# ubisoft/ubisoft-laforge-msmd

Hardware: AMD Instinct MI355X
Metric: FLAME frames/sec on 4s@16kHz clips (whole job; MSMD.forward motion-coefficient frames) (higher is better)
Workload: dtype bf16; 1 GPU; configs[1]: MSMD.forward, batch=32 x 4 s clips per GPU, wav2vec2-base encoder + 8-layer motion decoder, eval-mode, synthetic closed-form weights; batch_per_gpu=32, frames_per_clip=100, parallelism=dp1 (independent clips, no collective), launch=one hipGraph replay per step (the batch sits in the captured input buffers)

## Files before the change

include/msmd_hip.h:

```cpp
#ifndef MSMD_HIP_H
#define MSMD_HIP_H

#include <stdint.h>

#ifdef __cplusplus
extern "C" {
#endif

#define MSMD_F32 0
#define MSMD_BF16 1
#define MSMD_F16 2
#define MSMD_F16X2 3

#define MSMD_ACT_NONE 0
#define MSMD_ACT_GELU 1
#define MSMD_ACT_ELU 2

typedef void* msmd_stream_t;

int msmd_abi_version(void);
#define MSMD_GEMM_VARIANT(v) ((v) << 8)
#define MSMD_GEMM_WRITE_THROUGH (1 << 16)
#define MSMD_GEMM_PAIRED_STORES (1 << 17)
#define MSMD_GEMM_STAGGER (1 << 18)
// ... 105 lines not shown
                                    long q_bstride, long q_tstride, long k_bstride, long k_tstride, long v_bstride,
                                    long v_tstride, long o_bstride, long o_tstride, float scale, const uint8_t* mask,
                                    float p_drop, const unsigned long* rng_state, unsigned int site, int dtype,
                                    const void* const* prefetch_ptrs, const long* prefetch_bytes, int n_prefetch,
                                    msmd_stream_t stream);

int msmd_dropout(const void* x, const void* residual, void* y, long n, float p, const unsigned long* rng_state,
                 unsigned int site, int dtype, msmd_stream_t stream);

int msmd_attention_bwd(const void* Q, const void* K, const void* V, const void* dO, void* dQ, void* dK, void* dV,
                       int B, int H, int Tq, int Tk, long q_bstride, long q_tstride, long k_bstride,
                       long k_tstride, long v_bstride, long v_tstride, long do_bstride, long do_tstride,
                       long dq_bstride, long dq_tstride, long dk_bstride, long dk_tstride, long dv_bstride,
                       long dv_tstride, float scale, const uint8_t* mask, float p_drop,
                       const unsigned long* rng_state, unsigned int site, msmd_stream_t stream);

int msmd_pad_audio(const float* audio, float* out, int B, int L, int reflect_len, int replicate_len,
                   msmd_stream_t stream);

#define MSMD_CONV0_SPLITS 16
int msmd_conv0_stats(const float* audio, const float* w0, float* stats, double* ws, int B, int L, int reflect_len,
                     int replicate_len, int C, float eps, msmd_stream_t stream);

int msmd_conv0_gn_gelu(const float* audio, const float* w0, const float* stats, const float* gamma,
                       const float* beta, void* out, int B, int L, int reflect_len, int replicate_len,
                       int C, int out_dtype, msmd_stream_t stream);

int msmd_conv0_ln_gelu(const float* audio, const float* w0, const float* bias, const float* gamma, const float* beta,
                       void* out, int B, int L, int reflect_len, int replicate_len, int C, float eps, int out_dtype,
                       msmd_stream_t stream);

int msmd_interp_linear(const void* x, void* y, int B, int T_in, int T_crop, int T_out, int C, int dtype,
                       msmd_stream_t stream);

int msmd_group_pad(const void* x, void* y, int B, int T, int G, int Cg, int Cg_out, int pad, int dtype, int out_dtype,
                   msmd_stream_t stream);

int msmd_pos_conv(const void* x, const void* w, const float* bias, void* y, int B, int T, int G, int Cg, int kpos,
                  int dtype, msmd_stream_t stream);

int msmd_denoiser_pack_input(const float* motion, const float* eps, const float* c0, const float* c1,
                             const float* prev_motion, const float* indicator, void* feats, int N, int L,
                             int Lp, int dm, int Kpad, int motion_batch, int out_dtype, msmd_stream_t stream);

int msmd_denoiser_pack_input_guided(const float* motion, const float* eps, const float* c0, const float* c1,
                                    const float* prev_motion, const float* indicator, const unsigned char* guide_mask,
                                    const float* guide_values, void* feats, int N, int L, int Lp, int dm, int Kpad,
                                    int motion_batch, int out_dtype, msmd_stream_t stream);

int msmd_denoiser_prepare(const float* motion, const float* eps, const float* t0, const float* t1, const long* ts,
                          int n_steps, const float* prev_motion, long prev_motion_stride, const float* indicator,
                          void* feats, int N, int L, int Lp, int dm, int Kpad, const float* person_a, int cols_a,
                          const float* person_b, int cols_b, void* pf, int kp_person, const float* style,
                          long style_n, void* style_out, const void* emb_table, void* emb, int d,
                          const float* prev_audio, long prev_audio_stride, int Lpa, void* mem, long mem_stride,
                          int dtype, msmd_stream_t stream);
// ... 348 lines not shown
```

ubisoft-laforge-msmd_amd/csrc/audio.hip:

```cpp
#include "common.h"

__device__ __forceinline__ int pad_src(int j, int L, int r, int rep) {
  const int L1 = L + 2 * r, L2 = L1 + 2 * r;
  j -= rep;
  j = j < 0 ? 0 : (j >= L2 ? L2 - 1 : j);
  if (r > 0) {
    j -= r;
    j = j < 0 ? -j : (j >= L1 ? 2 * (L1 - 1) - j : j);
    j -= r;
    j = j < 0 ? -j : (j >= L ? 2 * (L - 1) - j : j);
  }
  return j;
}

__global__ void pad_audio_kernel(const float* __restrict__ a, float* __restrict__ out, int L, int Lp, int r, int rep) {
  const int b = blockIdx.y;
  for (int j = blockIdx.x * blockDim.x + threadIdx.x; j < Lp; j += gridDim.x * blockDim.x)
    out[(long)b * Lp + j] = a[(long)b * L + pad_src(j, L, r, rep)];
}

extern "C" int msmd_pad_audio(const float* audio, float* out, int B, int L, int reflect_len, int replicate_len,
                              msmd_stream_t stream) {
  if (B <= 0 || L <= 0 || reflect_len < 0 || replicate_len < 0 || reflect_len >= L) return 1;
  const int Lp = L + 4 * reflect_len + 2 * replicate_len;
  dim3 grid(min((Lp + 255) / 256, 1024), B), block(256);
  hipLaunchKernelGGL(pad_audio_kernel, grid, block, 0, (hipStream_t)stream, audio, out, L, Lp, reflect_len,
                     replicate_len);
  MSMD_RETURN_LAST();
}

#define C0_K 10
#define C0_S 5
#define C0_SPLITS 16
#define C0_NMOM 66

static bool conv0_geometry_ok(int B, int L, int reflect_len, int replicate_len) {
  if (B <= 0 || L <= 0 || reflect_len < 0 || replicate_len < 0 || reflect_len >= L) return false;
  return (long)L + 4L * reflect_len + 2L * replicate_len >= C0_K;
}


__global__ __launch_bounds__(256) void conv0_moments_partial(const float* __restrict__ audio, double* __restrict__ ws,
                                                             int L, int r, int rep, int T0, int pass) {
  __shared__ double red[4][C0_NMOM];
  const int b = blockIdx.y, split = blockIdx.x;
  const int per = (T0 + C0_SPLITS - 1) / C0_SPLITS;
  const int t_begin = split * per, t_end = min(T0, t_begin + per);
  double* out = ws + ((long)b * C0_SPLITS + split) * C0_NMOM;
  const float* xa = audio + (long)b * L;
  const int n_used = T0 * C0_S + C0_K - C0_S;
  const int n_mu = min(256, n_used);
  {
    const int j = (int)(((long)threadIdx.x * n_used) / n_mu);
    double v = threadIdx.x < n_mu ? (double)xa[pad_src(j, L, r, rep)] : 0.0;
    for (int o = 32; o > 0; o >>= 1) v += __shfl_xor(v, o, 64);
    if ((threadIdx.x & 63) == 0) red[threadIdx.x >> 6][0] = v;
    __syncthreads();
  }
  const float mu = (float)((red[0][0] + red[1][0] + red[2][0] + red[3][0]) / (double)n_mu);
  if (threadIdx.x == 0) out[0] = (double)mu;
  float m[C0_NMOM];
#pragma unroll
  for (int i = 0; i < C0_NMOM; ++i) m[i] = 0.f;
  for (int t = t_begin + threadIdx.x; t < t_end; t += 256) {
    float x[C0_K];
#pragma unroll
    for (int k = 0; k < C0_K; ++k) x[k] = xa[pad_src(t * C0_S + k, L, r, rep)] - mu;
#pragma unroll
    for (int k = 0; k < C0_K; ++k) {
      m[1 + k] += x[k];
#pragma unroll
      for (int k2 = k; k2 < C0_K; ++k2) {
        const int idx = 1 + C0_K + k * C0_K - (k * (k - 1)) / 2 + (k2 - k);
        m[idx] = fmaf(x[k], x[k2], m[idx]);
      }
    }
  }
#pragma unroll
  for (int i = 1; i < C0_NMOM; ++i) {
    double v = (double)m[i];
    for (int o = 32; o > 0; o >>= 1) v += __shfl_xor(v, o, 64);
    if ((threadIdx.x & 63) == 0) red[threadIdx.x >> 6][i] = v;
  }
  __syncthreads();
  if (threadIdx.x >= 1 && threadIdx.x < C0_NMOM)
    out[threadIdx.x] = red[0][threadIdx.x] + red[1][threadIdx.x] + red[2][threadIdx.x] + red[3][threadIdx.x];
}

__global__ void conv0_stats_finish(const double* __restrict__ ws, const float* __restrict__ w0,
                                   float* __restrict__ stats, int C, int T0, float eps) {
  __shared__ double mom[C0_NMOM];
  const int b = blockIdx.y;
  if (threadIdx.x < C0_NMOM) {
    double v = 0.0;
    for (int s = 0; s < C0_SPLITS; ++s) v += ws[((long)b * C0_SPLITS + s) * C0_NMOM + threadIdx.x];
    mom[threadIdx.x] = v;
  }
  __syncthreads();
  const int c = blockIdx.x * blockDim.x + threadIdx.x;
  if (c >= C) return;
  const double mu = ws[(long)b * C0_SPLITS * C0_NMOM];
  double w[C0_K], wsum = 0.0, ws1 = 0.0, q = 0.0;
  for (int k = 0; k < C0_K; ++k) { w[k] = (double)w0[c * C0_K + k]; wsum += w[k]; ws1 += w[k] * mom[1 + k]; }
  int idx = 1 + C0_K;
  for (int k = 0; k < C0_K; ++k)
    for (int k2 = k; k2 < C0_K; ++k2) q += (k2 == k ? 1.0 : 2.0) * w[k] * w[k2] * mom[idx++];
  const double mc = ws1 / T0;
  const double var = q / T0 - mc * mc;
  stats[((long)b * C + c) * 2 + 0] = (float)(mc + mu * wsum);
  stats[((long)b * C + c) * 2 + 1] = (float)(1.0 / sqrt(fmax(var, 0.0) + (double)eps));
}

extern "C" int msmd_conv0_stats(const float* audio, const float* w0, float* stats, double* ws, int B, int L,
                                int reflect_len, int replicate_len, int C, float eps, msmd_stream_t stream) {
  if (!conv0_geometry_ok(B, L, reflect_len, replicate_len) || C <= 0 || !ws) return 1;
  const int Lp = L + 4 * reflect_len + 2 * replicate_len;
  const int T0 = (Lp - C0_K) / C0_S + 1;
  hipStream_t st = (hipStream_t)stream;
  dim3 grid(C0_SPLITS, B);
  hipLaunchKernelGGL(conv0_moments_partial, grid, dim3(256), 0, st, audio, ws, L, reflect_len, replicate_len, T0, 1);
  hipLaunchKernelGGL(conv0_stats_finish, dim3((C + 255) / 256, B), dim3(256), 0, st, ws, w0, stats, C, T0, eps);
  MSMD_RETURN_LAST();
}

template <typename TO, bool SPLIT = false>
__global__ __launch_bounds__(256) void conv0_gn_gelu_kernel(const float* __restrict__ audio,
                                                            const float* __restrict__ w0,
                                                            const float* __restrict__ stats,
                                                            const float* __restrict__ gamma,
                                                            const float* __restrict__ beta, TO* __restrict__ out,
                                                            int L, int r, int rep, int C, int T0) {
  constexpr int FR = 64;
  __shared__ float xs[FR * C0_S + C0_K];
  const int b = blockIdx.y, t0 = blockIdx.x * FR;
  const int nt = min(FR, T0 - t0);
  const int ns = nt * C0_S + (C0_K - C0_S);
  for (int i = threadIdx.x; i < ns; i += 256) xs[i] = audio[(long)b * L + pad_src(t0 * C0_S + i, L, r, rep)];
  __syncthreads();
  const int grp = threadIdx.x >> 6, q = threadIdx.x & 63;
  for (int c0 = q * 8; c0 < C; c0 += 512) {
    float w[8][C0_K], sc[8], sh[8];
#pragma unroll
    for (int e = 0; e < 8; ++e) {
      const int c = c0 + e;
#pragma unroll
// ... 210 lines not shown
    }
  }
}

extern "C" int msmd_conv0_ln_gelu(const float* audio, const float* w0, const float* bias, const float* gamma,
                                  const float* beta, void* out, int B, int L, int reflect_len, int replicate_len,
                                  int C, float eps, int out_dtype, msmd_stream_t stream) {
  if (!conv0_geometry_ok(B, L, reflect_len, replicate_len) || C != 512) return 1;
  const int Lp = L + 4 * reflect_len + 2 * replicate_len;
  const int T0 = (Lp - C0_K) / C0_S + 1;
  dim3 grid((T0 + 63) / 64, B), block(256);
  return dispatch_dtype<float, f16_t, bf16_t>(out_dtype, [&](auto tag) {
    typedef MSMD_TAG_T(tag) TO;
    hipLaunchKernelGGL(conv0_ln_gelu_kernel<TO>, grid, block, 0, (hipStream_t)stream, audio, w0, bias, gamma, beta,
                       (TO*)out, L, reflect_len, replicate_len, T0, eps);
    MSMD_RETURN_LAST();
  });
}

template <typename T>
__global__ void interp_linear_kernel(const T* __restrict__ x, T* __restrict__ y, int T_in, int T_crop, int T_out,
                                     int C) {
  const int b = blockIdx.z, j = blockIdx.y;
  const float scale = (float)T_crop / (float)T_out;
  float src = fmaf(scale, (float)j + 0.5f, -0.5f);
  src = src < 0.f ? 0.f : src;
  int i0 = (int)src;
  i0 = i0 < T_crop - 1 ? i0 : T_crop - 1;
  const int i1 = i0 + 1 < T_crop ? i0 + 1 : T_crop - 1;
  const float w1 = src - (float)i0, w0 = 1.0f - w1;
  const T* p0 = x + ((long)b * T_in + i0) * C;
  const T* p1 = x + ((long)b * T_in + i1) * C;
  T* q = y + ((long)b * T_out + j) * C;
  for (int c = blockIdx.x * blockDim.x + threadIdx.x; c < C; c += gridDim.x * blockDim.x) {
#pragma clang fp contract(off)
    const float a0 = w0 * to_f32(p0[c]), a1 = w1 * to_f32(p1[c]);
    q[c] = from_f32<T>(a0 + a1);
  }
}

extern "C" int msmd_interp_linear(const void* x, void* y, int B, int T_in, int T_crop, int T_out, int C, int dtype,
                                  msmd_stream_t stream) {
  if (B <= 0 || T_in <= 0 || T_crop <= 0 || T_crop > T_in || T_out <= 0 || C <= 0) return 1;
  dim3 grid((C + 255) / 256, T_out, B), block(256);
  return dispatch_dtype<float, f16_t, bf16_t>(dtype, [&](auto tag) {
    typedef MSMD_TAG_T(tag) T;
    hipLaunchKernelGGL(interp_linear_kernel<T>, grid, block, 0, (hipStream_t)stream, (const T*)x, (T*)y, T_in, T_crop,
                       T_out, C);
    MSMD_RETURN_LAST();
  });
}

template <typename T, bool SPLIT>
__global__ void group_pad_kernel(const T* __restrict__ x, void* __restrict__ yv, int Tn, int G, int Cg, int Cgo,
                                 int pad) {
  const int b = blockIdx.z, g = blockIdx.y;
  const int Tp = Tn + 2 * pad;
  const long n = (long)Tp * Cgo;
  for (long i = blockIdx.x * blockDim.x + threadIdx.x; i < n; i += (long)gridDim.x * blockDim.x) {
    const int tp = (int)(i / Cgo), c = (int)(i % Cgo);
    const int t = tp - pad;
// ... 33 lines not shown
```

ubisoft-laforge-msmd_amd/csrc/common.h:

```cpp
#pragma once
#include <hip/hip_runtime.h>
#include <stdint.h>

#include "../../include/msmd_hip.h"

typedef __bf16 bf16_t;
typedef __bf16 bf16x8 __attribute__((ext_vector_type(8)));
typedef __bf16 bf16x4 __attribute__((ext_vector_type(4)));
typedef __bf16 bf16x2 __attribute__((ext_vector_type(2)));
typedef _Float16 f16_t;
typedef _Float16 f16x8 __attribute__((ext_vector_type(8)));
typedef _Float16 f16x4 __attribute__((ext_vector_type(4)));
typedef _Float16 f16x2 __attribute__((ext_vector_type(2)));
typedef float f32x4 __attribute__((ext_vector_type(4)));
typedef float f32x2 __attribute__((ext_vector_type(2)));
typedef float f32x16 __attribute__((ext_vector_type(16)));
typedef uint32_t u32x4 __attribute__((ext_vector_type(4)));
typedef uint32_t u32x2 __attribute__((ext_vector_type(2)));

struct __attribute__((packed, aligned(4))) F3 { float x, y, z; };
struct __attribute__((packed, aligned(4))) I3 { int a, b, c; };

#define MSMD_WAVE 64

// ... 162 lines not shown
}
__device__ __forceinline__ double wave_sum_f64(double v) {
#pragma unroll
  for (int o = 32; o > 0; o >>= 1) v += __shfl_xor(v, o, 64);
  return v;
}
__device__ __forceinline__ float wave_max(float v) {
#pragma unroll
  for (int o = 32; o > 0; o >>= 1) v = fmaxf(v, __shfl_xor(v, o, 64));
  return v;
}

__device__ __forceinline__ float block_sum(float v, float* red) {
  v = wave_sum(v);
  const int lane = threadIdx.x & 63, wid = threadIdx.x >> 6, nw = blockDim.x >> 6;
  __syncthreads();
  if (lane == 0) red[wid] = v;
  __syncthreads();
  float t = 0.f;
  for (int i = 0; i < nw; ++i) t += red[i];
  return t;
}

template <typename T> struct Elems16;
template <> struct Elems16<float> { static constexpr int n = 4; };
template <> struct Elems16<bf16_t> { static constexpr int n = 8; };
template <> struct Elems16<f16_t> { static constexpr int n = 8; };

template <typename T> struct TypeTag { typedef T type; };
template <typename T> struct DtypeCode;
template <> struct DtypeCode<float> { static constexpr int value = MSMD_F32; };
template <> struct DtypeCode<bf16_t> { static constexpr int value = MSMD_BF16; };
template <> struct DtypeCode<f16_t> { static constexpr int value = MSMD_F16; };
template <typename... Ts, typename F>
static int dispatch_dtype(int dtype, F&& f) {
  int r = 1;
  (void)((dtype == DtypeCode<Ts>::value && ((r = f(TypeTag<Ts>{})), true)) || ...);
  return r;
}
#define MSMD_TAG_T(tag) typename decltype(tag)::type
template <typename TI, typename TO> constexpr bool kStoragePair = sizeof(TI) == 4 || sizeof(TO) == 4 || __is_same(TI, TO);
```

ubisoft-laforge-msmd_amd/csrc/gemm.hip:

```cpp
#include "gemm_tiles.h"
#include <atomic>
#include <utility>

struct GemmArgs {
  const void* A; const void* W; const float* bias; const void* R; void* C;
  int M, N, K;
  long lda; int rows_per_batch; long a_batch_stride; long ldw, ldc, ldr;
  int act; int vec_ok; float inv_rpb;
  long strideA, strideW, strideC, strideBias, strideR;
  int mt, nt;
  int batch_inner; long strideA2, strideW2, strideC2;
  void* Z; float p_drop; const unsigned long* rng; unsigned site;
  int xn;
  int flags;
  const float* a_stats = nullptr; int a_nt = 0; const float* w_colsum = nullptr;
  const float* r_stats = nullptr; int r_nt = 0; const float* r_gamma = nullptr; const float* r_beta = nullptr;
  float* stats_out = nullptr; float ln_eps = 1e-5f;
  int stagger_ticks = 0;
};

enum : int {
  GF_WRITE_THROUGH = 1, GF_PAIRED_STORES = 2, GF_STAGGER = 4,
  GF_ACT_BWD = 8,
  GF_ONE_TILE = 16, GF_NO_256 = 32,
// ... 1990 lines not shown

extern "C" int msmd_gemm_actbwd(const void* A, const void* W, const void* Z, void* C, int M, int N, int K, int in_dtype, int out_dtype, long lda,
                                long ldw, int act, float p_drop, const unsigned long* rng_state, unsigned int site, msmd_stream_t stream) {
  if (!Z || in_dtype != out_dtype || (in_dtype != MSMD_BF16 && in_dtype != MSMD_F16) || (N & 3) || ((uintptr_t)Z & 7)) return 1;
  if (K % 64) return 1;
  GemmCall c;
  c.A = A; c.W = W; c.C = C; c.M = M; c.N = N; c.K = K; c.in_dtype = in_dtype; c.out_dtype = out_dtype;
  c.lda = lda; c.ldw = ldw; c.ldc = N; c.act = act & (0xffff | MSMD_GEMM_WRITE_THROUGH | MSMD_GEMM_PAIRED_STORES);
  c.z_out = const_cast<void*>(Z); c.p_drop = p_drop; c.rng = rng_state; c.site = site; c.internal_flags = GF_ACT_BWD;
  return gemm_run(gemm_plan, c, stream);
}

extern "C" int msmd_gemm_batched2(const void* A, const void* W, void* C, int M, int N, int K, int in_dtype, int out_dtype, long lda, long ldw,
                                  long ldc, int batch_outer, long strideA_o, long strideW_o, long strideC_o, int batch_inner, long strideA_i,
                                  long strideW_i, long strideC_i, msmd_stream_t stream) {
  GemmCall c;
  c.A = A; c.W = W; c.C = C; c.M = M; c.N = N; c.K = K; c.in_dtype = in_dtype; c.out_dtype = out_dtype;
  c.lda = lda; c.ldw = ldw; c.ldc = ldc; c.act = MSMD_ACT_NONE;
  c.batch = batch_outer; c.strideA = strideA_o; c.strideW = strideW_o; c.strideC = strideC_o;
  c.batch_inner = batch_inner; c.strideA2 = strideA_i; c.strideW2 = strideW_i; c.strideC2 = strideC_i;
  return gemm_run(gemm_plan, c, stream);
}

static bool conv_chain_table(ChainTable& t, int B, int T0, int C, int N, int n, const int* kernel, const int* stride, int flags) {
  if (B <= 0 || T0 <= 0 || C <= 0 || N <= 0 || n < 2 || n > 4 || !kernel || !stride || (N % 256)) return false;
  t = ChainTable{};
  t.n = n; t.nt = N / 256;
  t.per_block = (flags & MSMD_CONV_CHAIN_ROW_BLOCK_TICKETS) != 0;
  t.release = (flags & MSMD_CONV_CHAIN_RELEASE) != 0;
  long t_in = T0, c_in = C;
  int tickets = 0, counters = 0;
  for (int l = 0; l < n; ++l) {
    ChainProblem& q = t.pr[l];
    if (kernel[l] <= 0 || stride[l] <= 0 || t_in < kernel[l]) return false;
    const long t_out = (t_in - kernel[l]) / stride[l] + 1, M = (long)B * t_out, K = kernel[l] * c_in;
    if ((K % 64) || K < 128 || M >= (1L << 24)) return false;
    q.M = (int)M; q.K = (int)K; q.rows_per_batch = (int)t_out; q.inv_rpb = 1.0f / (float)t_out;
    q.lda = stride[l] * c_in; q.a_batch_stride = t_in * c_in;
    q.t_in = (int)t_in; q.stride = stride[l]; q.taps = kernel[l];
    q.mt = (int)((M + 255) / 256);
    q.ticket0 = tickets; q.cnt0 = counters;
    tickets += t.per_block ? q.mt : q.mt * t.nt;
    counters += q.mt;
    if (((long)(B - 1) * q.a_batch_stride + (t_out - 1) * q.lda + K) * 2 >= (1L << 32) || (long)N * K * 2 >= (1L << 32)) return false;
    t_in = t_out; c_in = N;
  }
// ... 58 lines not shown
```

ubisoft-laforge-msmd_amd/model.py:

```python
from __future__ import annotations

from types import SimpleNamespace

import torch
import torch.nn as nn

from . import init, ops, shapes, synth
from .blocks import Rows, add, materialise, norm, project
from .utils.model_common import ParamTree, PositionalEncoding, enc_dec_mask, sinusoid_table


def _cd(args) -> torch.dtype:
    name = getattr(args, "compute_dtype", "bf16")
    if name in ("bf16", torch.bfloat16):
        return torch.bfloat16
    if name in ("fp32", "float32", torch.float32):
        return torch.float32
    if name in ("f16x2", "split"):
        return torch.float32
    if name in ("fp16", "float16", "half", torch.float16):
        return torch.float16
    raise ValueError(f"Unknown compute dtype {name}!")


# ... 528 lines not shown
    @torch.no_grad()
    def extract_audio_768_feature(self, audio, frame_num=None):
        frame_num = frame_num or self.n_motions
        return self._audio_768(audio, frame_num, self.compute_dtype).float()

    @torch.no_grad()
    def forward(self, motion_feat, audio_or_feat, shape_feat, style_feat=None, prev_motion_feat=None,
                prev_audio_feat=None, time_step=None, indicator=None, train_with_CFG=True, keep_separate=False,
                eps=None):
        dtype = self.compute_dtype
        if self.use_style:
            assert style_feat is not None, "Missing style features!"
        batch_size = motion_feat.shape[0]
        net = self.denoising_net
        fused = net.prepares_fused(dtype) and not self.training
        if prev_audio_feat is None:
            prev_audio_feat = self.start_audio_feat.expand(batch_size, -1, -1)
        mem = None
        if audio_or_feat.ndim == 2:
            assert audio_or_feat.shape[1] == 16000 * self.n_motions / self.fps, \
                f"Incorrect audio length {audio_or_feat.shape[1]}"
            if fused:
                La, Lpa, d = self.n_motions, prev_audio_feat.shape[1], net.feature_dim
                h = self._audio_768(audio_or_feat, La, dtype)
                mem = torch.empty(batch_size, Lpa + La, d, device=self.device, dtype=dtype)
                audio_cd = mem[:, Lpa:]
                ops.gemm(h, *self._afm_packed(dtype), out=audio_cd, M=La, N=d, K=h.shape[-1], lda=h.shape[-1], ldc=d,
                         batch=batch_size, strideA=La * h.shape[-1], strideW=0, strideC=(Lpa + La) * d)
            else:
                audio_cd = self._audio_feat(audio_or_feat, self.n_motions, dtype)
            audio_feat_saved = audio_cd.float()
        elif audio_or_feat.ndim == 3:
            assert audio_or_feat.shape[1] == self.n_motions, f"Incorrect audio feature length {audio_or_feat.shape[1]}"
            audio_feat_saved = audio_or_feat
        else:
            raise ValueError(f"Incorrect audio input shape {audio_or_feat.shape}")
        audio_feat = audio_feat_saved
        if audio_or_feat.ndim != 2:
            audio_cd = None
        if shape_feat.ndim == 2:
            shape_feat = shape_feat.unsqueeze(1)
        if style_feat is not None and style_feat.ndim == 2:
            style_feat = style_feat.unsqueeze(1)
        if prev_motion_feat is None:
            prev_motion_feat = self.start_motion_feat.expand(batch_size, -1, -1)
        if len(self.guiding_conditions) > 0 and train_with_CFG:
            assert len(self.guiding_conditions) <= 2, "Only support 1 or 2 CFG conditions!"
            if len(self.guiding_conditions) == 1 or self.cfg_mode == "independent":
                null_cond_prob = 0.5 if len(self.guiding_conditions) >= 2 else 0.1
                if "style" in self.guiding_conditions:
                    mask_style = torch.rand(batch_size, device=self.device) < null_cond_prob
                    style_feat = torch.where(mask_style.view(-1, 1, 1),
                                             self.null_style_feat.expand(batch_size, -1, -1), style_feat)
                if "audio" in self.guiding_conditions:
# ... 130 lines not shown
```

ubisoft-laforge-msmd_amd/ops.py:

```python
from __future__ import annotations

import ctypes
import functools
import math
import os

import numpy as np
import torch
from torch.autograd.function import once_differentiable

from . import _lib

_HEADER = _lib.parse_constants()


def _h(*names):
    vals = tuple(_HEADER["MSMD_" + n] for n in names)
    return vals if len(vals) > 1 else vals[0]


F32, BF16, F16, F16X2 = _h("F32", "BF16", "F16", "F16X2")
SPLIT = "f16x2"


# ... 541 lines not shown

def dynamic_threshold_(res, L, ratio, dt_min, dt_max):
    _need_cuda(res)
    if res.dtype != torch.float32 or not res.is_contiguous():
        raise TypeError("dynamic_threshold_ takes a contiguous fp32 tensor")
    N, T_all, C = res.shape
    _lib.check(_lib.load().msmd_dynamic_threshold(_p(res), N, T_all, L, C, float(ratio), float(dt_min), float(dt_max),
                                                  _stream()), "msmd_dynamic_threshold")
    return res


def pad_audio(audio, reflect_len, replicate_len):
    lib = _lib.load()
    B, L = audio.shape
    out = torch.empty(B, L + 4 * reflect_len + 2 * replicate_len, device=audio.device, dtype=torch.float32)
    _lib.check(lib.msmd_pad_audio(_p(audio), _p(out), B, L, reflect_len, replicate_len, _stream()), "msmd_pad_audio")
    return out


def conv0_workspace(B, device):
    return torch.empty(B, CONV0_SPLITS, 66, device=device, dtype=torch.float64)


def conv0_gn_gelu(audio, w0, gamma, beta, reflect_len, replicate_len, out_dtype, eps=1e-5):
    lib = _lib.load()
    B, L = audio.shape
    C = w0.shape[0]
    Lp = L + 4 * reflect_len + 2 * replicate_len
    T0 = (Lp - 10) // 5 + 1
    stats = torch.empty(B, C, 2, device=audio.device, dtype=torch.float32)
    ws = conv0_workspace(B, audio.device)
    _lib.check(lib.msmd_conv0_stats(_p(audio), _p(w0), _p(stats), _p(ws), B, L, reflect_len, replicate_len, C, eps,
                                    _stream()), "msmd_conv0_stats")
    out = empty((B, T0, C), audio.device, out_dtype)
    _lib.check(lib.msmd_conv0_gn_gelu(_p(audio), _p(w0), _p(stats), _p(gamma), _p(beta), _p(out), B, L, reflect_len,
                                      replicate_len, C, _dt(out), _stream()), "msmd_conv0_gn_gelu")
    return out


def conv0_ln_gelu(audio, w0, bias, gamma, beta, reflect_len, replicate_len, out_dtype, eps=1e-5):
    lib = _lib.load()
    B, L = audio.shape
    C = w0.shape[0]
    Lp = L + 4 * reflect_len + 2 * replicate_len
    T0 = (Lp - 10) // 5 + 1
    out = torch.empty(B, T0, C, device=audio.device, dtype=out_dtype)
    _lib.check(lib.msmd_conv0_ln_gelu(_p(audio), _p(w0), _p(bias), _p(gamma), _p(beta), _p(out), B, L, reflect_len,
                                      replicate_len, C, eps, _dt(out), _stream()), "msmd_conv0_ln_gelu")
    return out


def interp_linear(x, t_out, t_crop=None):
    lib = _lib.load()
    B, T, C = x.shape
    t_crop = T if t_crop is None else min(int(t_crop), T)
    y = torch.empty(B, t_out, C, device=x.device, dtype=x.dtype)
    _lib.check(lib.msmd_interp_linear(_p(x), _p(y), B, T, t_crop, t_out, C, _dt(x), _stream()), "msmd_interp_linear")
    return y


def group_pad(x, groups, pad, cg_out=None, split=False):
    lib = _lib.load()
    B, T, C = x.shape
    cg = C // groups
    cg_out = cg if cg_out is None else cg_out
    y = empty((B, groups, T + 2 * pad, cg_out), x.device, SPLIT if split else x.dtype)
    _lib.check(lib.msmd_group_pad(_p(x), _p(y), B, T, groups, cg, cg_out, pad, _dt(x), _dt(y), _stream()),
               "msmd_group_pad")
    return y


def pos_conv(x, w, bias, groups, kpos=128):
    lib = _lib.load()
    _need_cuda(x)
    B, T, C = x.shape
    cg = C // groups
    if not (x.is_contiguous() and w.is_contiguous() and w.dtype == x.dtype and tuple(w.shape) == (groups, cg, kpos * cg)):
        raise TypeError("pos_conv takes contiguous x (B, T, G*Cg) and w (G, Cg, kpos*Cg) of one 16-bit dtype")
    if bias.dtype != torch.float32 or bias.numel() != C:
        raise TypeError("pos_conv takes an fp32 bias of G*Cg values")
    y = torch.empty_like(x)
# ... 1732 lines not shown
```

ubisoft-laforge-msmd_amd/training_script.py:

```python
from __future__ import annotations

import contextlib
import os

import numpy as np
import torch

from . import autograd as ag
from . import dp, ops, synth
from . import train_graph as tg


def load_loss_weights(args, device=None):
    w = {"noise": 1.0, "vert": float(args.l_vert), "vel": float(args.l_vel), "smooth": float(args.l_smooth),
         "head_angle": float(args.l_head_angle), "head_vel": float(args.l_head_vel),
         "head_smooth": float(args.l_head_smooth), "head_trans": float(args.l_head_trans)}
    if not args.use_vertex_space:
        w["vel"] *= 4.5e-8
        w["smooth"] *= 4e-7
    legacy = args.dataset_type[:9] == "HDTF_TFHP" or args.dataset_type == "flame_mead_ravdess"
    if not legacy and args.use_vertex_space:
        w["vert"] *= 1e-7
        w["vel"] *= 1e-7
        w["smooth"] *= 2e-8
# ... 290 lines not shown
            motion_in = ops.truncate_rows_(motion.float().clone().contiguous(), e32, 1, self.pad_replicate)
            indicator = (torch.arange(args.n_motions, device=self.device).expand(B, -1) < end_idx.unsqueeze(1)).float()
        else:
            audio_in, motion_in = audio, motion
            indicator = torch.ones(B, args.n_motions, device=self.device)
        ts = draws["t"][i] if "t" in draws else model.diffusion_sched.uniform_sample_t_device(B)
        eps = draws["eps"][i] if "eps" in draws else torch.randn_like(motion_in)
        ns, na = self._cfg_masks(draws, i, B)
        shape_in = torch.zeros_like(shape) if getattr(args, "do_ignore_shape", False) else shape
        return dict(style=style, end_idx=end_idx, audio_in=audio_in, motion_in=motion_in, indicator=indicator, ts=ts, eps=eps,
                    ns=ns, na=na, shape_in=shape_in)

    def _hand_off(self, batch, W0, audio_feat, dtype):
        model, n_prev = self.model, self.args.n_prev_motions
        if W0["end_idx"] is None:
            return W0["motion_in"][:, -n_prev:].detach(), audio_feat[:, -n_prev:].detach()
        audio = batch[0][0]
        with torch.no_grad():
            if ag.TrainNoise.active:
                prev_audio = tg.audio_feat_train(model, audio, model.n_motions, dtype).float()[:, -n_prev:]
            else:
                enc = model.audio_encoder
                chain, enc.conv_chain = enc.conv_chain, False
                try:
                    prev_audio = model.extract_audio_feature(audio)[:, -n_prev:]
                finally:
                    enc.conv_chain = chain
        return batch[1][0][:, -n_prev:], prev_audio

    def _loss_terms(self, i, W, target, prev_motion, shape, mu, logvar, terms, lw):
        args = self.args
        prev = prev_motion if i == 1 else None
        if self.vertex_space:
            pairs = tg.loss_vert_train(args, i == 0, shape, W["motion_in"], target, prev, self.coef_stats, self.flame,
                                       W["end_idx"]).items()
        else:
            tup = tg.loss_no_vert_train(args, i == 0, W["motion_in"], target, prev, W["end_idx"],
                                        halve=False)
            pairs = zip(("noise", "vel", "smooth", "head_angle", "head_vel", "head_smooth", "head_trans"),
                        [(v, 0.5) for v in tup[:6]] + [(tup[6], 1.0)])
        for key, val in pairs:
            val, sc = val if isinstance(val, tuple) else (val, 1.0)
            if val is not None and torch.is_tensor(val) and lw.get(key, 0) > 0:
                terms[key].append((val, sc))
        terms["kl_div"].append((tg.kl_train(mu, logvar), 1.0))

    def _two_windows_batched(self, batch, draws, trunc, cross, lw, dtype):
        model, se = self.model, self.style_enc
        audio_pair, motion_pair, shape = batch
        B = audio_pair[0].shape[0]
# ... 446 lines not shown
```

ubisoft-laforge-msmd_amd/utils/wav2vec2.py:

```python
from __future__ import annotations

from types import SimpleNamespace

import torch
import torch.nn as nn

from .. import ops, shapes, synth
from ..blocks import Rows, add, materialise, norm, project
from .model_common import ParamTree, pad_audio_plan

CONV_KERNEL = shapes.CONV_KERNEL
CONV_STRIDE = shapes.CONV_STRIDE


def compute_mask_indices(shape, mask_prob, mask_length, min_masks=0, rng=None):
    import numpy as np
    rng = np.random if rng is None else rng
    bsz, T = shape
    n_mask = max(min_masks, int(mask_prob * T / float(mask_length) + rng.rand()))
    spans = []
    for _ in range(bsz):
        lengths = np.full(n_mask, mask_length)
        if lengths.sum() == 0:
            lengths[0] = min(mask_length, T - 1)
# ... 85 lines not shown
            snap = os.path.join(repo, "snapshots", open(ref).read().strip())
            if _is_checkpoint_dir(snap):
                return snap
        for snap in sorted(glob.glob(os.path.join(repo, "snapshots", "*"))):
            if _is_checkpoint_dir(snap):
                return snap
    return None


def load_hf_state_dict(directory):
    import os
    st = os.path.join(directory, "model.safetensors")
    if os.path.isfile(st):
        from safetensors.torch import load_file
        return load_file(st, device="cpu")
    sd = torch.load(os.path.join(directory, "pytorch_model.bin"), map_location="cpu", weights_only=True)
    return sd.get("state_dict", sd) if isinstance(sd, dict) else sd


class Wav2Vec2Model(nn.Module):

    model_type = "wav2vec2"
    conv_chain = True

    def __init__(self, config=None):
        super().__init__()
        cfg = dict(num_hidden_layers=12, hidden_size=768, intermediate_size=3072, num_attention_heads=12,
                   conv_dim=512, num_conv_pos_embeddings=128, num_conv_pos_embedding_groups=16,
                   layer_norm_eps=1e-5, output_attentions=False,
                   feat_extract_norm="group", conv_bias=False, do_stable_layer_norm=False,
                   hidden_dropout=0.1, attention_dropout=0.1, activation_dropout=0.1, feat_proj_dropout=0.1,
                   layerdrop=0.1, apply_spec_augment=True, mask_time_prob=0.05, mask_time_length=10,
                   mask_time_min_masks=2)
        if config is not None:
            cfg.update({k: v for k, v in (config if isinstance(config, dict) else vars(config)).items() if v is not None})
        self.config = SimpleNamespace(**cfg)
        c = self.config
        if isinstance(c.conv_dim, (tuple, list)):
            c.conv_dim = int(c.conv_dim[0])
        if c.feat_extract_norm not in ("group", "layer"):
            raise ValueError(f"Unknown feat_extract_norm {c.feat_extract_norm!r}")
        tree = ParamTree(shapes.audio_encoder_shapes(c.num_hidden_layers, c.hidden_size, c.intermediate_size,
                                                     c.conv_dim, c.num_conv_pos_embeddings,
                                                     c.num_conv_pos_embedding_groups, c.feat_extract_norm,
                                                     c.conv_bias))
        for name, p in tree._parameters.items():
# ... 141 lines not shown
        self._packed, self._packed_dtype = P, (dtype, split)
        return P

    def feature_extractor_cl(self, audio, dtype, reflect_len=None, replicate_len=None, chain=True):
        P = self.pack_fe(dtype)
        if reflect_len is None:
            reflect_len, replicate_len = 0, 0
        eps = self.config.layer_norm_eps
        if self.config.feat_extract_norm == "layer":
            x = ops.conv0_ln_gelu(audio.float().contiguous(), P.w0, P.conv_b[0], *P.conv_ln[0], reflect_len,
                                  replicate_len, dtype, eps)
            for i, w in enumerate(P.conv_w):
                z = ops.conv1d_cl(x, w, P.conv_b[i + 1], kernel=CONV_KERNEL[i + 1], stride=CONV_STRIDE[i + 1])
                x = ops.layernorm(z, *P.conv_ln[i + 1], post_act=ops.ACT_GELU, eps=eps)
            return x
        if P.split:
            x = ops.conv0_gn_gelu(audio.float().contiguous(), P.w0, P.gn_g, P.gn_b, reflect_len, replicate_len,
                                  ops.SPLIT, eps)
            for i, w in enumerate(P.conv_w):
                last = i == len(P.conv_w) - 1
                x = ops.conv1d_cl(x, w, P.conv_b[i + 1], kernel=CONV_KERNEL[i + 1], stride=CONV_STRIDE[i + 1],
                                  act=ops.ACT_GELU, out_dtype=torch.float32 if last else ops.SPLIT)
            return x
        x = ops.conv0_gn_gelu(audio.float().contiguous(), P.w0, P.gn_g, P.gn_b, reflect_len, replicate_len, dtype, eps)
        first = 0
        if self.conv_chain and chain and len(P.conv_w) >= 4:
            outs = ops.conv_chain(x, P.conv_w[:4], P.conv_b[1:5], kernels=CONV_KERNEL[1:5], strides=CONV_STRIDE[1:5],
                                  act=ops.ACT_GELU)
            if outs is not None:
                x, first = outs[-1], 4
        for i, w in enumerate(P.conv_w):
            if i < first:
                continue
            x = ops.conv1d_cl(x, w, P.conv_b[i + 1], kernel=CONV_KERNEL[i + 1], stride=CONV_STRIDE[i + 1],
                              act=ops.ACT_GELU)
        return x

    def encode_features(self, x, dtype):
        P = self.pack(dtype)
        c = self.config
        B, T, _ = x.shape
        H, d, eps = c.num_attention_heads, c.hidden_size, c.layer_norm_eps
        scale = (d // H) ** -0.5
        pre = c.do_stable_layer_norm
        split = P.split and not pre
        fold = P.fold and ops.FOLD_LN
        h = ops.gemm(ops.layernorm(x, *P.fp_ln, eps=eps, split="only" if split else None), P.fp_w, P.fp_b)
# ... 58 lines not shown
```

Before: 883,400 frames/s.

## Fuse audio interpolation into feature-map GEMM and add LDS tree moment reduction

Adds an audio_junction kernel that performs the linear time interpolation of encoder features while staging A tiles into LDS for the feature-map GEMM, and also writes an fp32 copy. This removes the separate interp kernel, its intermediate tensor and the later .float() conversion. Separately, the conv0 moment reduction gains an LDS-based tree variant that replaces 65 sequential wave shuffles per thread with a shared-memory transpose plus partial tree sums. The new kernel uses a simple double-buffered loop with a full waitcnt, which may be slower than the tuned generic GEMM path.

```diff
diff --git a/include/msmd_hip.h b/include/msmd_hip.h
--- a/include/msmd_hip.h
+++ b/include/msmd_hip.h
@@ -151,6 +151,9 @@
 int msmd_conv0_stats(const float* audio, const float* w0, float* stats, double* ws, int B, int L, int reflect_len,
                      int replicate_len, int C, float eps, msmd_stream_t stream);
 
+int msmd_conv0_stats_lds(const float* audio, const float* w0, float* stats, double* ws, int B, int L, int reflect_len,
+                         int replicate_len, int C, float eps, msmd_stream_t stream);
+
 int msmd_conv0_gn_gelu(const float* audio, const float* w0, const float* stats, const float* gamma,
                        const float* beta, void* out, int B, int L, int reflect_len, int replicate_len,
                        int C, int out_dtype, msmd_stream_t stream);
@@ -161,6 +164,9 @@
 
 int msmd_interp_linear(const void* x, void* y, int B, int T_in, int T_crop, int T_out, int C, int dtype,
                        msmd_stream_t stream);
+
+int msmd_audio_junction(const void* x, const void* W, const float* bias, void* C, float* C32, int B, int T_in, int T_crop,
+                        int T_out, int N, int K, long c_batch_stride, int dtype, msmd_stream_t stream);
 
 int msmd_group_pad(const void* x, void* y, int B, int T, int G, int Cg, int Cg_out, int pad, int dtype, int out_dtype,
                    msmd_stream_t stream);
diff --git a/ubisoft-laforge-msmd_amd/csrc/audio.hip b/ubisoft-laforge-msmd_amd/csrc/audio.hip
--- a/ubisoft-laforge-msmd_amd/csrc/audio.hip
+++ b/ubisoft-laforge-msmd_amd/csrc/audio.hip
@@ -40,13 +40,13 @@
 }
 
 
-__global__ __launch_bounds__(256) void conv0_moments_partial(const float* __restrict__ audio, double* __restrict__ ws,
-                                                             int L, int r, int rep, int T0, int pass) {
-  __shared__ double red[4][C0_NMOM];
+__device__ __forceinline__ void conv0_thread_moments(const float* __restrict__ audio, double* __restrict__ ws,
+                                                     double (&red)[4][C0_NMOM], float (&m)[C0_NMOM], double*& out, int L,
+                                                     int r, int rep, int T0) {
   const int b = blockIdx.y, split = blockIdx.x;
   const int per = (T0 + C0_SPLITS - 1) / C0_SPLITS;
   const int t_begin = split * per, t_end = min(T0, t_begin + per);
-  double* out = ws + ((long)b * C0_SPLITS + split) * C0_NMOM;
+  out = ws + ((long)b * C0_SPLITS + split) * C0_NMOM;
   const float* xa = audio + (long)b * L;
   const int n_used = T0 * C0_S + C0_K - C0_S;
   const int n_mu = min(256, n_used);
@@ -59,7 +59,6 @@
   }
   const float mu = (float)((red[0][0] + red[1][0] + red[2][0] + red[3][0]) / (double)n_mu);
   if (threadIdx.x == 0) out[0] = (double)mu;
-  float m[C0_NMOM];
 #pragma unroll
   for (int i = 0; i < C0_NMOM; ++i) m[i] = 0.f;
   for (int t = t_begin + threadIdx.x; t < t_end; t += 256) {
@@ -76,11 +75,58 @@
       }
     }
   }
+}
+
+__global__ __launch_bounds__(256) void conv0_moments_partial(const float* __restrict__ audio, double* __restrict__ ws,
+                                                             int L, int r, int rep, int T0, int pass) {
+  __shared__ double red[4][C0_NMOM];
+  float m[C0_NMOM];
+  double* out;
+  conv0_thread_moments(audio, ws, red, m, out, L, r, rep, T0);
 #pragma unroll
   for (int i = 1; i < C0_NMOM; ++i) {
     double v = (double)m[i];
     for (int o = 32; o > 0; o >>= 1) v += __shfl_xor(v, o, 64);
     if ((threadIdx.x & 63) == 0) red[threadIdx.x >> 6][i] = v;
+  }
+  __syncthreads();
+  if (threadIdx.x >= 1 && threadIdx.x < C0_NMOM)
+    out[threadIdx.x] = red[0][threadIdx.x] + red[1][threadIdx.x] + red[2][threadIdx.x] + red[3][threadIdx.x];
+}
+
+#define C0_TREE_HALF 33
+#define C0_LEAF_LD 68
+__global__ __launch_bounds__(256) void conv0_moments_partial_lds(const float* __restrict__ audio, double* __restrict__ ws,
+                                                                 int L, int r, int rep, int T0) {
+  __shared__ double red[4][C0_NMOM];
+  __shared__ float leaf[4][C0_TREE_HALF][C0_LEAF_LD];
+  float m[C0_NMOM];
+  double* out;
+  conv0_thread_moments(audio, ws, red, m, out, L, r, rep, T0);
+  const int lane = threadIdx.x & 63, wid = threadIdx.x >> 6;
+#pragma unroll
+  for (int h = 0; h < 2; ++h) {
+    constexpr int HALF = C0_TREE_HALF;
+    const int first = 1 + h * HALF, n = h ? C0_NMOM - 1 - HALF : HALF;
+    if (h) __syncthreads();
+#pragma unroll
+    for (int i = 0; i < HALF; ++i)
+      if (i < n) leaf[wid][i][lane] = m[first + i];
+    __syncthreads();
+    for (int task = lane; task < 4 * n; task += 64) {
+      const int i = task >> 2, j = task & 3;
+      double x[16];
+#pragma unroll
+      for (int u = 0; u < 16; ++u) x[u] = (double)leaf[wid][i][j + 4 * u];
+#pragma unroll
+      for (int o = 8; o > 0; o >>= 1)
+#pragma unroll
+        for (int u = 0; u < o; ++u) x[u] += x[u + o];
+      double v = x[0];
+      v += __shfl_xor(v, 2, 64);
+      v += __shfl_xor(v, 1, 64);
+      if (j == 0) red[wid][first + i] = v;
+    }
   }
   __syncthreads();
   if (threadIdx.x >= 1 && threadIdx.x < C0_NMOM)
@@ -111,16 +157,29 @@
   stats[((long)b * C + c) * 2 + 1] = (float)(1.0 / sqrt(fmax(var, 0.0) + (double)eps));
 }
 
-extern "C" int msmd_conv0_stats(const float* audio, const float* w0, float* stats, double* ws, int B, int L,
-                                int reflect_len, int replicate_len, int C, float eps, msmd_stream_t stream) {
+static int conv0_stats_launch(bool lds_trees, const float* audio, const float* w0, float* stats, double* ws, int B, int L,
+                              int reflect_len, int replicate_len, int C, float eps, msmd_stream_t stream) {
   if (!conv0_geometry_ok(B, L, reflect_len, replicate_len) || C <= 0 || !ws) return 1;
   const int Lp = L + 4 * reflect_len + 2 * replicate_len;
   const int T0 = (Lp - C0_K) / C0_S + 1;
   hipStream_t st = (hipStream_t)stream;
   dim3 grid(C0_SPLITS, B);
-  hipLaunchKernelGGL(conv0_moments_partial, grid, dim3(256), 0, st, audio, ws, L, reflect_len, replicate_len, T0, 1);
+  if (lds_trees)
+    hipLaunchKernelGGL(conv0_moments_partial_lds, grid, dim3(256), 0, st, audio, ws, L, reflect_len, replicate_len, T0);
+  else
+    hipLaunchKernelGGL(conv0_moments_partial, grid, dim3(256), 0, st, audio, ws, L, reflect_len, replicate_len, T0, 1);
   hipLaunchKernelGGL(conv0_stats_finish, dim3((C + 255) / 256, B), dim3(256), 0, st, ws, w0, stats, C, T0, eps);
   MSMD_RETURN_LAST();
+}
+
+extern "C" int msmd_conv0_stats(const float* audio, const float* w0, float* stats, double* ws, int B, int L,
+                                int reflect_len, int replicate_len, int C, float eps, msmd_stream_t stream) {
+  return conv0_stats_launch(false, audio, w0, stats, ws, B, L, reflect_len, replicate_len, C, eps, stream);
+}
+
+extern "C" int msmd_conv0_stats_lds(const float* audio, const float* w0, float* stats, double* ws, int B, int L,
+                                    int reflect_len, int replicate_len, int C, float eps, msmd_stream_t stream) {
+  return conv0_stats_launch(true, audio, w0, stats, ws, B, L, reflect_len, replicate_len, C, eps, stream);
 }
 
 template <typename TO, bool SPLIT = false>
@@ -377,21 +436,12 @@
 __global__ void interp_linear_kernel(const T* __restrict__ x, T* __restrict__ y, int T_in, int T_crop, int T_out,
                                      int C) {
   const int b = blockIdx.z, j = blockIdx.y;
-  const float scale = (float)T_crop / (float)T_out;
-  float src = fmaf(scale, (float)j + 0.5f, -0.5f);
-  src = src < 0.f ? 0.f : src;
-  int i0 = (int)src;
-  i0 = i0 < T_crop - 1 ? i0 : T_crop - 1;
-  const int i1 = i0 + 1 < T_crop ? i0 + 1 : T_crop - 1;
-  const float w1 = src - (float)i0, w0 = 1.0f - w1;
-  const T* p0 = x + ((long)b * T_in + i0) * C;
-  const T* p1 = x + ((long)b * T_in + i1) * C;
+  const InterpTaps t = interp_taps(j, T_crop, T_out);
+  const T* p0 = x + ((long)b * T_in + t.i0) * C;
+  const T* p1 = x + ((long)b * T_in + t.i1) * C;
   T* q = y + ((long)b * T_out + j) * C;
-  for (int c = blockIdx.x * blockDim.x + threadIdx.x; c < C; c += gridDim.x * blockDim.x) {
-#pragma clang fp contract(off)
-    const float a0 = w0 * to_f32(p0[c]), a1 = w1 * to_f32(p1[c]);
-    q[c] = from_f32<T>(a0 + a1);
-  }
+  for (int c = blockIdx.x * blockDim.x + threadIdx.x; c < C; c += gridDim.x * blockDim.x)
+    q[c] = from_f32<T>(interp_blend(t, to_f32(p0[c]), to_f32(p1[c])));
 }
 
 extern "C" int msmd_interp_linear(const void* x, void* y, int B, int T_in, int T_crop, int T_out, int C, int dtype,
diff --git a/ubisoft-laforge-msmd_amd/csrc/common.h b/ubisoft-laforge-msmd_amd/csrc/common.h
--- a/ubisoft-laforge-msmd_amd/csrc/common.h
+++ b/ubisoft-laforge-msmd_amd/csrc/common.h
@@ -208,6 +208,23 @@
   return t;
 }
 
+struct InterpTaps { int i0, i1; float w0, w1; };
+__device__ __forceinline__ InterpTaps interp_taps(int j, int T_crop, int T_out) {
+  const float scale = (float)T_crop / (float)T_out;
+  float src = fmaf(scale, (float)j + 0.5f, -0.5f);
+  src = src < 0.f ? 0.f : src;
+  int i0 = (int)src;
+  i0 = i0 < T_crop - 1 ? i0 : T_crop - 1;
+  const int i1 = i0 + 1 < T_crop ? i0 + 1 : T_crop - 1;
+  const float w1 = src - (float)i0;
+  return {i0, i1, 1.0f - w1, w1};
+}
+__device__ __forceinline__ float interp_blend(const InterpTaps& t, float x0, float x1) {
+#pragma clang fp contract(off)
+  const float a0 = t.w0 * x0, a1 = t.w1 * x1;
+  return a0 + a1;
+}
+
 template <typename T> struct Elems16;
 template <> struct Elems16<float> { static constexpr int n = 4; };
 template <> struct Elems16<bf16_t> { static constexpr int n = 8; };
diff --git a/ubisoft-laforge-msmd_amd/csrc/gemm.hip b/ubisoft-laforge-msmd_amd/csrc/gemm.hip
--- a/ubisoft-laforge-msmd_amd/csrc/gemm.hip
+++ b/ubisoft-laforge-msmd_amd/csrc/gemm.hip
@@ -2036,6 +2036,111 @@
   return gemm_run(gemm_plan, c, stream);
 }
 
+struct JunctionArgs {
+  const void* x; const void* W; const float* bias; void* C; float* C32;
+  int B, T_in, T_crop, T_out, N, K;
+  long c_bstride;
+};
+
+template <typename TI>
+__global__ __launch_bounds__(256) void audio_junction_kernel(const JunctionArgs a) {
+  constexpr int BM = 64, BN = 64, KS = 2, TILE = 64 * 128, STAGE = KS * 2 * TILE;
+  extern __shared__ __attribute__((aligned(16))) unsigned char smem[];
+  const int mt = (a.T_out + BM - 1) / BM, nt = (a.N + BN - 1) / BN;
+  const int grp = ((int)blockIdx.x >> 3) / nt * 8 + (blockIdx.x & 7);
+  if (grp >= mt * a.B) return;
+  const int tid = threadIdx.x, z = grp / mt, m0 = (grp % mt) * BM, n0 = (((int)blockIdx.x >> 3) % nt) * BN;
+  const int nk = a.K / 64, ns = (nk + KS - 1) / KS;
+
+  GemmArgs g{};
+  g.M = a.T_out; g.N = a.N; g.K = a.K; g.ldw = a.K; g.rows_per_batch = a.T_out;
+  TileSrc<bf16_t, 0, BN, 4> wsrc;
+  wsrc.set(g, (const bf16_t*)a.W, (const bf16_t*)a.W, 0, n0, tid);
+
+  const int ch = tid & 7;
+  int row[2];
+  InterpTaps tap[2];
+  const TI* p0[2];
+  const TI* p1[2];
+#pragma unroll
+  for (int r = 0; r < 2; ++r) {
+    row[r] = r * 32 + (tid >> 3);
+    tap[r] = interp_taps(min(m0 + row[r], a.T_out - 1), a.T_crop, a.T_out);
+    p0[r] = (const TI*)a.x + ((long)z * a.T_in + tap[r].i0) * a.K + ch * 8;
+    p1[r] = (const TI*)a.x + ((long)z * a.T_in + tap[r].i1) * a.K + ch * 8;
+  }
+  typedef typename Vec8T<TI>::type V8;
+  u32x4 ra[KS][2][2];
+  auto load_step = [&](int s, int buf) {
+#pragma unroll
+    for (int kk = 0; kk < KS; ++kk) {
+      const int kt = min(s * KS + kk, nk - 1);
+#pragma unroll
+      for (int r = 0; r < 2; ++r) {
+        ra[kk][r][0] = *(const u32x4*)(p0[r] + kt * 64);
+        ra[kk][r][1] = *(const u32x4*)(p1[r] + kt * 64);
+      }
+      wsrc.issue(smem + buf * STAGE + kk * 2 * TILE + TILE, kt, tid);
+    }
+  };
+
+  const FragLane l = frag_lane<BM, BN, 2, 2>(tid);
+  f32x4 acc[2][2];
+  zero_acc(acc);
+  load_step(0, 0);
+  for (int s = 0; s < ns; ++s) {
+    unsigned char* st = smem + (s & 1) * STAGE;
+#pragma unroll
+    for (int kk = 0; kk < KS; ++kk)
+#pragma unroll
+      for (int r = 0; r < 2; ++r) {
+        const V8 x0 = __builtin_bit_cast(V8, ra[kk][r][0]), x1 = __builtin_bit_cast(V8, ra[kk][r][1]);
+        TI o[8];
+#pragma unroll
+        for (int e = 0; e < 8; ++e) o[e] = from_f32<TI>(interp_blend(tap[r], to_f32(x0[e]), to_f32(x1[e])));
+        *(V8*)(st + kk * 2 * TILE + lds_off(row[r], ch)) = V8{o[0], o[1], o[2], o[3], o[4], o[5], o[6], o[7]};
+      }
+    asm volatile("s_waitcnt vmcnt(0) lgkmcnt(0)" ::: "memory");
+    __syncthreads();
+    if (s + 1 < ns) load_step(s + 1, (s + 1) & 1);
+#pragma unroll
+    for (int kk = 0; kk < KS; ++kk)
+      if (s * KS + kk < nk) k_tile_mma<TI, 2, 2>(st + kk * 2 * TILE, st + kk * 2 * TILE + TILE, l, acc);
+  }
+
+  typedef typename Vec4T<TI>::type V4;
+#pragma unroll
+  for (int j = 0; j < 2; ++j) {
+    const int m = m0 + l.wm + j * 16 + l.fr;
+    if (m >= a.T_out) continue;
+#pragma unroll
+    for (int i = 0; i < 2; ++i) {
+      const int n = n0 + l.wn + i * 16 + l.fq * 4;
+      if (n >= a.N) continue;
+      const f32x4 bv = a.bias ? *(const f32x4*)(a.bias + n) : f32x4{0.f, 0.f, 0.f, 0.f};
+      const V4 o = pack4<TI>(acc[i][j][0] + bv[0], acc[i][j][1] + bv[1], acc[i][j][2] + bv[2], acc[i][j][3] + bv[3]);
+      *(V4*)((TI*)a.C + z * a.c_bstride + (long)m * a.N + n) = o;
+      *(f32x4*)(a.C32 + ((long)z * a.T_out + m) * a.N + n) = f32x4{(float)o[0], (float)o[1], (float)o[2], (float)o[3]};
+    }
+  }
+}
+
+extern "C" int msmd_audio_junction(const void* x, const void* W, const float* bias, void* C, float* C32, int B, int T_in, int T_crop,
+                                   int T_out, int N, int K, long c_batch_stride, int dtype, msmd_stream_t stream) {
+  if (!x || !W || !C || !C32 || B <= 0 || T_in <= 0 || T_crop <= 0 || T_crop > T_in || T_out <= 0 || N <= 0 || (N & 3) || K <= 0 ||
+      (K % 64) || c_batch_stride < (long)T_out * N || (c_batch_stride & 3))
+    return 1;
+  if (((uintptr_t)x & 15) || ((uintptr_t)W & 15) || ((uintptr_t)bias & 15) || ((uintptr_t)C & 7) || ((uintptr_t)C32 & 15)) return 1;
+  const JunctionArgs a{x, W, bias, C, C32, B, T_in, T_crop, T_out, N, K, c_batch_stride};
+  const long groups = (long)((T_out + 63) / 64) * B, wgs = (groups + 7) / 8 * 8 * ((N + 63) / 64);
+  if (wgs > 0x7fffffffL) return 1;
+  const dim3 grid((unsigned)wgs);
+  constexpr int lds = 2 * 2 * 2 * 64 * 128;
+  return dispatch_dtype<f16_t, bf16_t>(dtype, [&](auto tag) {
+    return gemm_launch_kernel<audio_junction_kernel<MSMD_TAG_T(tag)>>(grid, 256, lds, (hipStream_t)stream, a);
+  });
+}
+
 static bool conv_chain_table(ChainTable& t, int B, int T0, int C, int N, int n, const int* kernel, const int* stride, int flags) {
   if (B <= 0 || T0 <= 0 || C <= 0 || N <= 0 || n < 2 || n > 4 || !kernel || !stride || (N % 256)) return false;
   t = ChainTable{};
diff --git a/ubisoft-laforge-msmd_amd/model.py b/ubisoft-laforge-msmd_amd/model.py
--- a/ubisoft-laforge-msmd_amd/model.py
+++ b/ubisoft-laforge-msmd_amd/model.py
@@ -574,14 +574,19 @@
                 f"Incorrect audio length {audio_or_feat.shape[1]}"
             if fused:
                 La, Lpa, d = self.n_motions, prev_audio_feat.shape[1], net.feature_dim
-                h = self._audio_768(audio_or_feat, La, dtype)
                 mem = torch.empty(batch_size, Lpa + La, d, device=self.device, dtype=dtype)
                 audio_cd = mem[:, Lpa:]
-                ops.gemm(h, *self._afm_packed(dtype), out=audio_cd, M=La, N=d, K=h.shape[-1], lda=h.shape[-1], ldc=d,
-                         batch=batch_size, strideA=La * h.shape[-1], strideW=0, strideC=(Lpa + La) * d)
+                if getattr(self, "fused_junction", True):
+                    h = self.audio_encoder.encode(audio_or_feat, self.fps, frame_num=La * 2, dtype=dtype, pad=True)
+                    audio_feat_saved = ops.audio_junction(h, *self._afm_packed(dtype), audio_cd, La)
+                else:
+                    h = self._audio_768(audio_or_feat, La, dtype)
+                    ops.gemm(h, *self._afm_packed(dtype), out=audio_cd, M=La, N=d, K=h.shape[-1], lda=h.shape[-1], ldc=d,
+                             batch=batch_size, strideA=La * h.shape[-1], strideW=0, strideC=(Lpa + La) * d)
+                    audio_feat_saved = audio_cd.float()
             else:
                 audio_cd = self._audio_feat(audio_or_feat, self.n_motions, dtype)
-            audio_feat_saved = audio_cd.float()
+                audio_feat_saved = audio_cd.float()
         elif audio_or_feat.ndim == 3:
             assert audio_or_feat.shape[1] == self.n_motions, f"Incorrect audio feature length {audio_or_feat.shape[1]}"
             audio_feat_saved = audio_or_feat
diff --git a/ubisoft-laforge-msmd_amd/ops.py b/ubisoft-laforge-msmd_amd/ops.py
--- a/ubisoft-laforge-msmd_amd/ops.py
+++ b/ubisoft-laforge-msmd_amd/ops.py
@@ -587,16 +587,25 @@
     return torch.empty(B, CONV0_SPLITS, 66, device=device, dtype=torch.float64)
 
 
-def conv0_gn_gelu(audio, w0, gamma, beta, reflect_len, replicate_len, out_dtype, eps=1e-5):
+def conv0_stats(audio, w0, reflect_len, replicate_len, eps=1e-5, lds=False):
+    lib = _lib.load()
+    B, C = audio.shape[0], w0.shape[0]
+    stats = torch.empty(B, C, 2, device=audio.device, dtype=torch.float32)
+    ws = conv0_workspace(B, audio.device)
+    name = "msmd_conv0_stats_lds" if lds else "msmd_conv0_stats"
+    _lib.check(getattr(lib, name)(_p(audio), _p(w0), _p(stats), _p(ws), B, audio.shape[1], reflect_len, replicate_len, C,
+                                  eps, _stream()), name)
+    return stats, ws
+
+
+def conv0_gn_gelu(audio, w0, gamma, beta, reflect_len, replicate_len, out_dtype, eps=1e-5, stats_lds=False):
     lib = _lib.load()
     B, L = audio.shape
     C = w0.shape[0]
     Lp = L + 4 * reflect_len + 2 * replicate_len
     T0 = (Lp - 10) // 5 + 1
-    stats = torch.empty(B, C, 2, device=audio.device, dtype=torch.float32)
-    ws = conv0_workspace(B, audio.device)
-    _lib.check(lib.msmd_conv0_stats(_p(audio), _p(w0), _p(stats), _p(ws), B, L, reflect_len, replicate_len, C, eps,
-                                    _stream()), "msmd_conv0_stats")
+    stats, _ = conv0_stats(audio, w0, reflect_len, replicate_len, eps,
+                           lds=stats_lds and out_dtype in (torch.bfloat16, torch.float16))
     out = empty((B, T0, C), audio.device, out_dtype)
     _lib.check(lib.msmd_conv0_gn_gelu(_p(audio), _p(w0), _p(stats), _p(gamma), _p(beta), _p(out), B, L, reflect_len,
                                       replicate_len, C, _dt(out), _stream()), "msmd_conv0_gn_gelu")
@@ -622,6 +631,22 @@
     y = torch.empty(B, t_out, C, device=x.device, dtype=x.dtype)
     _lib.check(lib.msmd_interp_linear(_p(x), _p(y), B, T, t_crop, t_out, C, _dt(x), _stream()), "msmd_interp_linear")
     return y
+
+
+def audio_junction(x, w, bias, out, t_out, t_crop=None):
+    lib = _lib.load()
+    _need_cuda(x, w, out)
+    B, T, K = x.shape
+    N = w.shape[0]
+    if x.dtype not in (torch.bfloat16, torch.float16) or w.dtype != x.dtype or out.dtype != x.dtype:
+        raise TypeError("audio_junction takes one 16-bit type for x, w and out")
+    if not x.is_contiguous() or not w.is_contiguous() or tuple(out.shape) != (B, t_out, N) or out.stride(2) != 1 or out.stride(1) != N:
+        raise ValueError("audio_junction: contiguous x / w, out (B, t_out, N) with rows N apart")
+    t_crop = T if t_crop is None else min(int(t_crop), T)
+    out32 = torch.empty(B, t_out, N, device=x.device, dtype=torch.float32)
+    _lib.check(lib.msmd_audio_junction(_p(x), _p(w), _p(bias), _p(out), _p(out32), B, T, t_crop, t_out, N, K,
+                                       out.stride(0) if B > 1 else t_out * N, _dt(x), _stream()), "msmd_audio_junction")
+    return out32
 
 
 def group_pad(x, groups, pad, cg_out=None, split=False):
diff --git a/ubisoft-laforge-msmd_amd/training_script.py b/ubisoft-laforge-msmd_amd/training_script.py
--- a/ubisoft-laforge-msmd_amd/training_script.py
+++ b/ubisoft-laforge-msmd_amd/training_script.py
@@ -336,10 +336,11 @@
             else:
                 enc = model.audio_encoder
                 chain, enc.conv_chain = enc.conv_chain, False
+                lds, enc.conv0_stats_lds = enc.conv0_stats_lds, False
                 try:
                     prev_audio = model.extract_audio_feature(audio)[:, -n_prev:]
                 finally:
-                    enc.conv_chain = chain
+                    enc.conv_chain, enc.conv0_stats_lds = chain, lds
         return batch[1][0][:, -n_prev:], prev_audio
 
     def _loss_terms(self, i, W, target, prev_motion, shape, mu, logvar, terms, lw):
diff --git a/ubisoft-laforge-msmd_amd/utils/wav2vec2.py b/ubisoft-laforge-msmd_amd/utils/wav2vec2.py
--- a/ubisoft-laforge-msmd_amd/utils/wav2vec2.py
+++ b/ubisoft-laforge-msmd_amd/utils/wav2vec2.py
@@ -131,6 +131,7 @@
 
     model_type = "wav2vec2"
     conv_chain = True
+    conv0_stats_lds = True
 
     def __init__(self, config=None):
         super().__init__()
@@ -318,7 +319,8 @@
                 x = ops.conv1d_cl(x, w, P.conv_b[i + 1], kernel=CONV_KERNEL[i + 1], stride=CONV_STRIDE[i + 1],
                                   act=ops.ACT_GELU, out_dtype=torch.float32 if last else ops.SPLIT)
             return x
-        x = ops.conv0_gn_gelu(audio.float().contiguous(), P.w0, P.gn_g, P.gn_b, reflect_len, replicate_len, dtype, eps)
+        x = ops.conv0_gn_gelu(audio.float().contiguous(), P.w0, P.gn_g, P.gn_b, reflect_len, replicate_len, dtype, eps,
+                              stats_lds=chain and self.conv0_stats_lds)
         first = 0
         if self.conv_chain and chain and len(P.conv_w) >= 4:
             outs = ops.conv_chain(x, P.conv_w[:4], P.conv_b[1:5], kernels=CONV_KERNEL[1:5], strides=CONV_STRIDE[1:5],
```

Measured after the change: 890,100 frames/s (median of 6 runs). Within noise of the previous version (+0.8%).
